# Ghostish/Open3DSOT

Measured on AMD Instinct MI355X. Metric: template/search pairs/sec (fwd+bwd), BAT KITTI-Car 512/1024 pts, higher is better.
Workload: dtype f32; 1 GPU; BAT_Car.yaml KITTI-Car, template 512 / search 1024 pts, batch 48 per GPU, fwd+bwd+Adam, fp32; global_batch=48, parallelism=dp1, fused_kernels=True, hip_graph=True, rccl_world_size=1

## Files before the change

### open3dsot_amd/csrc/compact.hip

```cpp
#include <cstdlib>
#include "o3d_common.hpp"

namespace {

__global__ __launch_bounds__(256) void compact_count_kernel(const int32_t* __restrict__ idx, long nslots, int ns,
                                                            int32_t* __restrict__ ball_cnt) {
    const long s = (long)blockIdx.x * 256 + threadIdx.x;
    const int lane = threadIdx.x & 63;
    const int v = s < nslots ? idx[s] : -1;
    const int base = lane & ~(ns - 1), k = lane - base;
    const int first = __shfl(v, base, 64);
    const unsigned long long m = __ballot(v != first);
    const unsigned long long seg = ns == 64 ? ~0ull : (((1ull << ns) - 1) << base);
    const unsigned long long other = m & seg;
    if (k == 0 && s < nslots) ball_cnt[s / ns] = other ? (63 - __clzll((long long)other)) - base + 1 : 1;
}

__global__ __launch_bounds__(1024) void compact_scan_kernel(const int32_t* __restrict__ ball_cnt, int n,
                                                            int col_base, int32_t* __restrict__ ball_off,
                                                            int32_t* __restrict__ meta) {
    __shared__ int sh[1024];
    const int per = (n + 1023) / 1024;
    const int i0 = threadIdx.x * per;
    int local = 0;
    for (int i = i0; i < i0 + per && i < n; ++i) local += ball_cnt[i];
    sh[threadIdx.x] = local;
    __syncthreads();
    for (int off = 1; off < 1024; off <<= 1) {
        const int v = (int)threadIdx.x >= off ? sh[threadIdx.x - off] : 0;
        __syncthreads();
        sh[threadIdx.x] += v;
        __syncthreads();
    }
    int run = col_base + sh[threadIdx.x] - local;
    for (int i = i0; i < i0 + per && i < n; ++i) {
        ball_off[i] = run;
        run += ball_cnt[i];
    }
    if (threadIdx.x == 1023) {
        const int tot = sh[1023];
        meta[0] = (tot + 255) & ~255;
        meta[1] = tot;
        meta[2] = n;
        meta[3] = 0;
    }
}

__global__ __launch_bounds__(256) void compact_fill_kernel(const int32_t* __restrict__ idx, long nslots, int ns,
                                                           int npoint, int ld, int col_base, int pt_base,
                                                           int ball_base, int dummy_ball,
                                                           const int32_t* __restrict__ ball_cnt,
                                                           const int32_t* __restrict__ ball_off,
                                                           const int32_t* __restrict__ meta,
                                                           int32_t* __restrict__ gp, int32_t* __restrict__ cball,
                                                           float* __restrict__ cw) {
    if (blockIdx.x == gridDim.x - 1) {
        const int q = meta[1] + threadIdx.x;
        if (q < meta[0]) { gp[col_base + q] = 0; cball[col_base + q] = dummy_ball; cw[col_base + q] = 0.f; }
        return;
    }
    const long s = (long)blockIdx.x * 256 + threadIdx.x;
    if (s >= nslots) return;
    const int ball = (int)(s / ns), k = (int)(s - (long)ball * ns);
    const int cnt = ball_cnt[ball];
    if (k >= cnt) return;
    const int q = ball_off[ball] + k;
    gp[q] = pt_base + (ball / npoint) * ld + idx[s];
    cball[q] = ball_base + ball;
    cw[q] = k == 0 ? (float)(1 + ns - cnt) : 1.f;
}

template <bool CENTERS, bool DIRECT = false>
__global__ __launch_bounds__(256) void expand_c_kernel(const float* __restrict__ Z, long ldz,
                                                       const int32_t* __restrict__ gp,
                                                       const int32_t* __restrict__ cball,
                                                       const float* __restrict__ cw,
                                                       const float* __restrict__ centers,
                                                       const float* __restrict__ W0, int ldw, int C0,
                                                       const int32_t* __restrict__ meta, long start1, long ldp,
                                                       float* __restrict__ Y0, float* __restrict__ part,
                                                       const float* __restrict__ stat_c) {
    const int q0 = blockIdx.x * 256;
    const int seg = (start1 > 0 && q0 >= start1) ? 1 : 0;
// ... 78 lines not shown
}

template <int POOL_CH>
__global__ __launch_bounds__(256) void pool_c_kernel(const float* __restrict__ Y, long ldp,
                                                     const float* __restrict__ scale,
                                                     const float* __restrict__ shift,
                                                     const int32_t* __restrict__ ball_off,
                                                     const int32_t* __restrict__ ball_cnt, int C, int seg1_ball,
                                                     int np0, int np1, int nballs, float* __restrict__ out,
                                                     int32_t* __restrict__ argq, float* __restrict__ yarg) {
    const int e = threadIdx.x & 7;
    int ball = blockIdx.x * 32 + (threadIdx.x >> 3);
    const bool live = ball < nballs;
    if (!live) ball = nballs - 1;
    const int q0 = ball_off[ball], q1 = q0 + ball_cnt[ball];
    const int c0 = blockIdx.y * POOL_CH;
    if (ball >= seg1_ball) { scale += C; shift += C; }
    constexpr int PU = 4;
    float v[POOL_CH][PU], sc[POOL_CH], sf[POOL_CH];
#pragma unroll
    for (int cc = 0; cc < POOL_CH; ++cc) {
        const int c = c0 + cc < C ? c0 + cc : C - 1;
        const float* y = Y + (long)c * ldp;
#pragma unroll
        for (int i = 0; i < PU; ++i) {
            const int q = q0 + e + 8 * i;
            v[cc][i] = y[q < q1 ? q : q1 - 1];
        }
        sc[cc] = scale[c];
        sf[cc] = shift[c];
    }
    float rbest[POOL_CH], ryb[POOL_CH];
    int rbq[POOL_CH];
#pragma unroll
    for (int cc = 0; cc < POOL_CH; ++cc) {
        float best = -INFINITY, yb = 0.f;
        int bq = 0x7fffffff;
#pragma unroll
        for (int i = 0; i < PU; ++i) {
            const int q = q0 + e + 8 * i;
            const float n = fmaf(v[cc][i], sc[cc], sf[cc]);
            if (q < q1 && n > best) { best = n; bq = q; yb = v[cc][i]; }
        }
        if (q1 - q0 > 8 * PU) {
            const float* y = Y + (long)(c0 + cc < C ? c0 + cc : C - 1) * ldp;
            for (int q = q0 + e + 8 * PU; q < q1; q += 8) {
                const float w = y[q], n = fmaf(w, sc[cc], sf[cc]);
                if (n > best) { best = n; bq = q; yb = w; }
            }
        }
        {
            const float ob = dpp_f<0xB1>(best), oy = dpp_f<0xB1>(yb);
            const int oq = dpp_i<0xB1>(bq);
            if (ob > best || (ob == best && oq < bq)) { best = ob; bq = oq; yb = oy; }
        }
        {
            const float ob = dpp_f<0x4E>(best), oy = dpp_f<0x4E>(yb);
            const int oq = dpp_i<0x4E>(bq);
            if (ob > best || (ob == best && oq < bq)) { best = ob; bq = oq; yb = oy; }
        }
        {
            const float ob = dpp_f<0x141>(best), oy = dpp_f<0x141>(yb);
            const int oq = dpp_i<0x141>(bq);
            if (ob > best || (ob == best && oq < bq)) { best = ob; bq = oq; yb = oy; }
        }
        rbest[cc] = best; ryb[cc] = yb; rbq[cc] = bq;
    }
    if (live && e == 0) {
#pragma unroll
        for (int cc = 0; cc < POOL_CH; ++cc) {
            const int c = c0 + cc;
            if (c < C) {
                const long o = pool_index(c, ball, C, seg1_ball, np0, np1);
                out[o] = fmaxf(rbest[cc], 0.f);
                if (argq) { argq[o] = rbq[cc]; yarg[o] = ryb[cc]; }
            }
        }
    }
}

constexpr int PT_CH = 32, PT_COLS = 128, PT_OVER = 32, PT_LD = PT_COLS + PT_OVER + 3;
constexpr int PT_RB = 32, PT_RLD = PT_CH + 1;

__device__ __forceinline__ void pool_t_item(const float* __restrict__ Y, long ldp,
                                            const float* __restrict__ scale, const float* __restrict__ shift,
                                            const int32_t* __restrict__ ball_off,
                                            const int32_t* __restrict__ ball_cnt,
                                            const int32_t* __restrict__ cball,
                                            const int32_t* __restrict__ meta, long start1, int C,
                                            int seg1_ball, int np0, int np1, int nballs,
                                            float* __restrict__ out, int32_t* __restrict__ argq,
                                            float* __restrict__ yarg, const long q0, const int c0, float* pt_tile) {
    int* pt_off = reinterpret_cast<int*>(pt_tile + PT_CH * PT_LD);
    int* pt_cnt = pt_off + PT_COLS;
    int* pt_ob = pt_cnt + PT_COLS;
    float* pt_res = reinterpret_cast<float*>(pt_ob + PT_COLS);
    const int seg = (start1 > 0 && q0 >= start1) ? 1 : 0;
    const long sbase = seg ? start1 : 0;
    if (q0 - sbase >= meta[4 * seg]) return;
    const long qend = sbase + meta[4 * seg + 1];
    if (q0 >= qend) return;
    int bfirst = cball[q0];
    if (ball_off[bfirst] < q0) ++bfirst;
    const long qlast = (q0 + PT_COLS < qend ? q0 + PT_COLS : qend) - 1;
    const int blast = cball[qlast];
    const int nb = blast - bfirst + 1;
    const int np = seg ? np1 : np0;
    const long segbase = seg ? (long)seg1_ball * C : 0;
    const int ball0 = seg ? seg1_ball : 0;
    constexpr int F4 = (PT_COLS + PT_OVER) / 4;
    constexpr int NLD = PT_CH * F4 / 256;
    static_assert(PT_CH * F4 % 256 == 0, "tile loads must divide evenly over the workgroup");
    {
        float4 v[NLD];
        int bo = 0, bc = 0;
        if ((int)threadIdx.x < nb) { bo = ball_off[bfirst + threadIdx.x]; bc = ball_cnt[bfirst + threadIdx.x]; }
#pragma unroll
        for (int u = 0; u < NLD; ++u) {
            const int i = threadIdx.x + 256 * u;
            const int r = i / F4, f = i - r * F4;
            long q = q0 + 4 * f;
            if (q + 4 > ldp) q = ldp - 4;
            v[u] = *reinterpret_cast<const float4*>(&Y[(long)(c0 + r) * ldp + q]);
        }
        __builtin_amdgcn_sched_barrier(0);
#pragma unroll
        for (int u = 0; u < NLD; ++u) {
            const int i = threadIdx.x + 256 * u;
            const int r = i / F4, f = i - r * F4;
            float* d = &pt_tile[r * PT_LD + 4 * f];
            d[0] = v[u].x; d[1] = v[u].y; d[2] = v[u].z; d[3] = v[u].w;
        }
        if ((int)threadIdx.x < PT_COLS) {
            const int local = bfirst + (int)threadIdx.x - ball0;
            const int b = local / np, j = local - b * np;
            pt_off[threadIdx.x] = bo;
            pt_cnt[threadIdx.x] = bc;
            pt_ob[threadIdx.x] = (int)(segbase + (long)b * C * np + j);
        }
    }
    const int lane = threadIdx.x & 63, wave = threadIdx.x >> 6;
    const int ch = lane & (PT_CH - 1), half = lane / PT_CH;
    constexpr int BPW = 64 / PT_CH;
    const float sc = scale[seg * C + c0 + ch], sf = shift[seg * C + c0 + ch];
    __syncthreads();
    const float* row = &pt_tile[ch * PT_LD];
    const int wj = threadIdx.x & 31, wc = threadIdx.x >> 5;
    for (int j0 = 0; j0 < nb; j0 += PT_RB) {
#pragma unroll 1
        for (int t = 0; t < PT_RB / 4; t += BPW) {
            const int jl = j0 + wave * (PT_RB / 4) + t + half;
            if (jl - half >= nb) break;
            const bool has = jl < nb;
            const int off = has ? pt_off[jl] : 0, cnt = has ? pt_cnt[jl] : 0;
            const int rel = (int)(off - q0);
            float best = -INFINITY, yb = 0.f;
            int bq = 0x7fffffff;
            for (int k = 0; k < cnt; k += 4) {
                const float w0 = row[rel + k], w1 = row[rel + k + 1], w2 = row[rel + k + 2], w3 = row[rel + k + 3];
                const float n0 = fmaf(w0, sc, sf), n1 = fmaf(w1, sc, sf), n2 = fmaf(w2, sc, sf), n3 = fmaf(w3, sc, sf);
                if (n0 > best) { best = n0; bq = off + k; yb = w0; }
                if (k + 1 < cnt && n1 > best) { best = n1; bq = off + k + 1; yb = w1; }
                if (k + 2 < cnt && n2 > best) { best = n2; bq = off + k + 2; yb = w2; }
                if (k + 3 < cnt && n3 > best) { best = n3; bq = off + k + 3; yb = w3; }
            }
            if (has) {
                float* r = &pt_res[(jl - j0) * PT_RLD + ch];
                r[0] = fmaxf(best, 0.f);
                r[PT_RB * PT_RLD] = __int_as_float(bq);
                r[2 * PT_RB * PT_RLD] = yb;
            }
        }
        __syncthreads();
        if (j0 + wj < nb) {
            const int ob = pt_ob[j0 + wj];
#pragma unroll
            for (int cc = wc; cc < PT_CH; cc += 8) {
                const long o = (long)ob + (long)(c0 + cc) * np;
                const float* r = &pt_res[wj * PT_RLD + cc];
                out[o] = r[0];
                if (argq) { argq[o] = __float_as_int(r[PT_RB * PT_RLD]); yarg[o] = r[2 * PT_RB * PT_RLD]; }
            }
        }
        __syncthreads();
    }
}

constexpr int PT_GRID = 4096;
__global__ __launch_bounds__(256) void pool_t_kernel(const float* __restrict__ Y, long ldp,
                                                     const float* __restrict__ scale, const float* __restrict__ shift,
                                                     const int32_t* __restrict__ ball_off,
                                                     const int32_t* __restrict__ ball_cnt,
                                                     const int32_t* __restrict__ cball,
                                                     const int32_t* __restrict__ meta, long start1, int C,
                                                     int seg1_ball, int np0, int np1, int nballs,
                                                     float* __restrict__ out, int32_t* __restrict__ argq,
                                                     float* __restrict__ yarg) {
    extern __shared__ float pt_tile[];
    const int ngrp = C / PT_CH;
    const int n0 = (meta[1] + PT_COLS - 1) / PT_COLS;
    const int n1 = start1 > 0 ? (meta[5] + PT_COLS - 1) / PT_COLS : 0;
    const long items = (long)(n0 + n1) * ngrp;
    for (long it = blockIdx.x; it < items; it += gridDim.x) {
        const int ch = (int)(it / ngrp), cg = (int)(it - (long)ch * ngrp);
        const long q0 = ch < n0 ? (long)ch * PT_COLS : start1 + (long)(ch - n0) * PT_COLS;
        pool_t_item(Y, ldp, scale, shift, ball_off, ball_cnt, cball, meta, start1, C, seg1_ball, np0, np1, nballs, out, argq, yarg, q0,
                    cg * PT_CH, pt_tile);
        __syncthreads();
    }
}

__global__ __launch_bounds__(256) void zero_cols_kernel(float* __restrict__ D, long ldp,
                                                        const int32_t* __restrict__ meta, long start1) {
    const long q = ((long)blockIdx.x * 256 + threadIdx.x) * 4;
    if (q >= ldp) return;
    const int seg = (start1 > 0 && q >= start1) ? 1 : 0;
    if (q - (seg ? start1 : 0) >= meta[4 * seg]) return;
    *reinterpret_cast<float4*>(&D[(long)blockIdx.y * ldp + q]) = make_float4(0.f, 0.f, 0.f, 0.f);
}

__global__ __launch_bounds__(256) void pool_bwd_partials_c_kernel(const float* __restrict__ dOut,
                                                                  const float* __restrict__ out,
                                                                  const float* __restrict__ yarg,
                                                                  const float* __restrict__ mean, int C,
                                                                  int nballs, int seg1_ball, int np0, int np1,
                                                                  float* __restrict__ part,
                                                                  const int32_t* __restrict__ argq,
                                                                  float* __restrict__ D, long ldp) {
    __shared__ float sh[2][4];
    const int c = blockIdx.x, seg = blockIdx.y, k = blockIdx.z;
    const int s0 = seg ? seg1_ball : 0, s1 = seg ? nballs : seg1_ball;
    const int share = (s1 - s0 + POOL_BWD_SPLIT - 1) / POOL_BWD_SPLIT;
    const int b0 = s0 + k * share, b1 = min(b0 + share, s1);
    const float mu = mean[seg * C + c];
    float s = 0.f, q = 0.f;
    for (int ball = b0 + threadIdx.x; ball < b1; ball += 256) {
        const long o = pool_index(c, ball, C, seg1_ball, np0, np1);
        const bool pos = out[o] > 0.f;
        const float g = pos ? dOut[o] : 0.f;
        if (D && pos) D[(long)c * ldp + argq[o]] = g;
        s += g;
        q += g * (yarg[o] - mu);
    }
#pragma unroll
    for (int m = 32; m >= 1; m >>= 1) { s += __shfl_xor(s, m, 64); q += __shfl_xor(q, m, 64); }
    if ((threadIdx.x & 63) == 0) { sh[0][threadIdx.x >> 6] = s; sh[1][threadIdx.x >> 6] = q; }
    __syncthreads();
    if (threadIdx.x == 0) {
        const long row = (long)seg * POOL_BWD_SPLIT + k;
        part[(row * 2 + 0) * C + c] = (sh[0][0] + sh[0][1]) + (sh[0][2] + sh[0][3]);
        part[(row * 2 + 1) * C + c] = (sh[1][0] + sh[1][1]) + (sh[1][2] + sh[1][3]);
    }
}

constexpr int PBD_COLS = 512, PBD_CH = 8, PBD_BALLS = 128, PBD_GRID = 4096;

struct PoolGrad { const float* p; long sb, sc; };

struct PoolBwdDense {
    PoolGrad g0, g1;
    const float* out; const int32_t* argq; const float* yarg; const float* mean; const int32_t* cball; const int32_t* ball_off;
    const int32_t* meta; long start1, ldp; int C, dummy_ball, seg1_ball, np0, np1;
    float* D; float* part;
};

__device__ __forceinline__ void pool_bwd_dense_item(const PoolBwdDense& a, const long q0, const int c0, float2 (&stg)[PBD_CH][PBD_BALLS],
                                                    int& sh_hi) {
    const PoolGrad g0 = a.g0, g1 = a.g1;
    const float* __restrict__ out = a.out; const int32_t* __restrict__ argq = a.argq; const float* __restrict__ yarg = a.yarg;
    const float* __restrict__ mean = a.mean; const int32_t* __restrict__ cball = a.cball;
    const int32_t* __restrict__ ball_off = a.ball_off; const int32_t* __restrict__ meta = a.meta;
    const long start1 = a.start1, ldp = a.ldp;
    const int C = a.C, dummy_ball = a.dummy_ball, seg1_ball = a.seg1_ball, np0 = a.np0, np1 = a.np1;
    float* __restrict__ D = a.D; float* __restrict__ part = a.part;
    const long chunk = q0 / PBD_COLS;
    const int seg = (start1 > 0 && q0 >= start1) ? 1 : 0;
    const long local0 = q0 - (seg ? start1 : 0);
    const int qi = threadIdx.x & 127, half = threadIdx.x >> 7;
    const long q = q0 + 4 * qi;
    const int live = meta[4 * seg];
    const int b_lo = cball[q0];
    const int4 cb = *reinterpret_cast<const int4*>(&cball[q]);
    if (threadIdx.x == 0) sh_hi = -1;
    if (local0 >= live) return;
    const int ncols = (int)min((long)PBD_COLS, live - local0);
    const bool mine = 4 * qi < ncols;
    __syncthreads();
    if (half == 0) {
        int hi = cb.x;
        hi = cb.y != dummy_ball ? cb.y : hi;
        hi = cb.z != dummy_ball ? cb.z : hi;
// ... 341 lines not shown
        if (T)
            for (int j = threadIdx.x; j < npoint; j += 256) {
                const int b0 = ball_off[bbase + j], b1 = b0 + ball_cnt[bbase + j];
                const int s0 = b0 > lo ? b0 : lo, s1 = b1 < hi ? b1 : hi;
                if (s0 >= s1) continue;
                float t[CS];
#pragma unroll
                for (int c = 0; c < CS; ++c) t[c] = 0.f;
                for (int q = s0; q < s1; ++q)
#pragma unroll
                    for (int c = 0; c < CS; ++c) t[c] += dy[c * CH + (q - lo)];
#pragma unroll
                for (int c = 0; c < CS; ++c) tacc[c * npoint + j] += t[c];
            }
    }
    __syncthreads();
    for (int i = threadIdx.x; i < CS * ld; i += 256) {
        const int c = i / ld, n = i - c * ld;
        if (c0 + c < C0) S[(long)(c0 + c) * lds_row + pbase + n] = sacc[i];
    }
    if (T)
        for (int i = threadIdx.x; i < CS * npoint; i += 256) {
            const int c = i / npoint, j = i - c * npoint;
            if (c0 + c < C0) T[(long)(c0 + c) * nballs + bbase + j] = tacc[i];
        }
}

__global__ __launch_bounds__(1024) void center_term_kernel(const float* __restrict__ T,
                                                           const float* __restrict__ centers, int nballs, int ldw,
                                                           float* __restrict__ dW, float* __restrict__ out = nullptr,
                                                           int ncols = 0) {
    __shared__ float red[16][3];
    const int c = blockIdx.x, tid = threadIdx.x;
    const float* t = T + (long)c * nballs;
    float s0 = 0.f, s1 = 0.f, s2 = 0.f;
    for (int ball = tid; ball < nballs; ball += 1024) {
        const float v = t[ball];
        s0 = fmaf(v, centers[3 * ball], s0);
        s1 = fmaf(v, centers[3 * ball + 1], s1);
        s2 = fmaf(v, centers[3 * ball + 2], s2);
    }
#pragma unroll
    for (int off = 32; off >= 1; off >>= 1) {
        s0 += __shfl_xor(s0, off, 64);
        s1 += __shfl_xor(s1, off, 64);
        s2 += __shfl_xor(s2, off, 64);
    }
    if ((tid & 63) == 0) { red[tid >> 6][0] = s0; red[tid >> 6][1] = s1; red[tid >> 6][2] = s2; }
    __syncthreads();
    if (tid < 3) {
        float a = 0.f;
#pragma unroll
        for (int w = 0; w < 16; ++w) a += red[w][tid];
        if (out) out[(long)c * ncols + tid] = dW[(long)c * ldw + tid] - a;
        else dW[(long)c * ldw + tid] -= a;
    }
    if (out)
        for (int k = 3 + tid; k < ncols; k += 1024) out[(long)c * ncols + k] = dW[(long)c * ldw + k];
}

struct PackSeg { const float* xyz; const float* feats; int N, ld; };

__global__ __launch_bounds__(256) void pack_points_kernel(PackSeg s0, PackSeg s1, int B, int nxyz, int C, float inv_radius,
                                                          long ldz, float* __restrict__ X0) {
    const long col = (long)blockIdx.x * 256 + threadIdx.x;
    if (col >= ldz) return;
    const int r = blockIdx.y;
    const long base1 = (long)B * s0.ld;
    const bool second = col >= base1;
    const PackSeg sg = second ? s1 : s0;
    const long local = second ? col - base1 : col;
    const int b = (int)(local / sg.ld), n = (int)(local - (long)b * sg.ld);
    float v = 0.f;
    if (n < sg.N) {
        if (r < nxyz) v = sg.xyz[((long)b * sg.N + n) * 3 + r] * inv_radius;
        else if (r < nxyz + C) v = sg.feats[((long)b * C + (r - nxyz)) * sg.N + n];
    }
    X0[(long)r * ldz + col] = v;
}

}

static bool pow2(int v) { return v > 0 && (v & (v - 1)) == 0; }
constexpr long O3D_MAX_BALLS = 1L << 20;

extern "C" int o3d_compact_build(const int32_t* idx, int B, int npoint, int ns, int ld, int col_base, int pt_base,
                                 int ball_base, int dummy_ball, int32_t* ball_cnt, int32_t* ball_off, int32_t* gp,
                                 int32_t* cball, float* cw, int32_t* meta, void* stream) {
    const long nballs = (long)B * npoint, nslots = nballs * ns;
    if (!idx || !ball_cnt || !ball_off || !gp || !cball || !cw || !meta || B <= 0 || npoint <= 0 || ns < 1 ||
        ns > 64 || !pow2(ns) || nballs > O3D_MAX_BALLS || nslots % 256 != 0 || ld <= 0 || col_base < 0 || col_base % 256 != 0)
        return O3D_EINVAL;
    hipStream_t s = o3d_stream(stream);
    const int blocks = (int)(nslots / 256);
    hipLaunchKernelGGL(compact_count_kernel, dim3(blocks), dim3(256), 0, s, idx, nslots, ns, ball_cnt);
    hipLaunchKernelGGL(compact_scan_kernel, dim3(1), dim3(1024), 0, s, ball_cnt, (int)nballs, col_base, ball_off, meta);
    hipLaunchKernelGGL(compact_fill_kernel, dim3(blocks + 1), dim3(256), 0, s, idx, nslots, ns, npoint, ld, col_base,
                       pt_base, ball_base, dummy_ball, ball_cnt, ball_off, meta, gp, cball, cw);
    return o3d_launch_status();
}

namespace {
template <int CPW>
__global__ __launch_bounds__(256) void dw0_xyz_kernel(const float* __restrict__ dN, const float* __restrict__ Y0, long ldp,
                                                      const float* __restrict__ A1, const float* __restrict__ A2,
                                                      const float* __restrict__ A3, const int32_t* __restrict__ gp,
                                                      const int32_t* __restrict__ cball, const float* __restrict__ cw,
                                                      const float* __restrict__ X, long ldz,
                                                      const float* __restrict__ centers,
                                                      const int32_t* __restrict__ meta, long start1, int C0,
                                                      float* __restrict__ part) {
    const long q0 = (long)blockIdx.x * 256;
    const int seg = (start1 > 0 && q0 >= start1) ? 1 : 0;
    float* prow = part + (long)blockIdx.x * C0 * 3;
    if (q0 - (seg ? start1 : 0) >= meta[4 * seg]) {
        for (int i = threadIdx.x; i < C0 * 3; i += 256) prow[i] = 0.f;
        return;
    }
    const int lane = threadIdx.x & 63, wave = threadIdx.x >> 6;
    const long q = q0 + 4 * lane;
    const int4 id = *reinterpret_cast<const int4*>(&gp[q]);
    const int4 bj = *reinterpret_cast<const int4*>(&cball[q]);
    const float4 w = *reinterpret_cast<const float4*>(&cw[q]);
    const int ids[4] = {id.x, id.y, id.z, id.w}, bb[4] = {bj.x, bj.y, bj.z, bj.w};
    const float wv[4] = {w.x, w.y, w.z, w.w};
    float rel[4][3];
#pragma unroll
    for (int t = 0; t < 4; ++t)
#pragma unroll
        for (int k = 0; k < 3; ++k)
            rel[t][k] = wv[t] != 0.f ? X[(long)k * ldz + ids[t]] - centers[(long)bb[t] * 3 + k] : 0.f;
    const float* a1 = A1 + seg * C0;
    const float* a2 = A2 + seg * C0;
    const float* a3 = A3 + seg * C0;
    for (int cbase = 0; cbase < C0; cbase += 4 * CPW) {
        float acc[CPW][3];
        float4 d[CPW], y[CPW];
#pragma unroll
        for (int i = 0; i < CPW; ++i) {
            const int c = cbase + wave + 4 * i;
            const int cc = c < C0 ? c : C0 - 1;
            d[i] = *reinterpret_cast<const float4*>(&dN[(long)cc * ldp + q]);
            y[i] = *reinterpret_cast<const float4*>(&Y0[(long)cc * ldp + q]);
        }
#pragma unroll
        for (int i = 0; i < CPW; ++i) {
            const int c = cbase + wave + 4 * i;
            const int cc = c < C0 ? c : C0 - 1;
            const float k1 = a1[cc], k2 = a2[cc], k3 = a3[cc];
            const float dv[4] = {d[i].x, d[i].y, d[i].z, d[i].w}, yv[4] = {y[i].x, y[i].y, y[i].z, y[i].w};
            float s0 = 0.f, s1 = 0.f, s2 = 0.f;
#pragma unroll
            for (int t = 0; t < 4; ++t) {
                const float dy = wv[t] != 0.f ? fmaf(k1, dv[t], wv[t] * fmaf(k2, yv[t], k3)) : 0.f;
                s0 = fmaf(dy, rel[t][0], s0); s1 = fmaf(dy, rel[t][1], s1); s2 = fmaf(dy, rel[t][2], s2);
            }
            acc[i][0] = s0; acc[i][1] = s1; acc[i][2] = s2;
        }
#pragma unroll
        for (int i = 0; i < CPW; ++i) {
            const int c = cbase + wave + 4 * i;
#pragma unroll
            for (int k = 0; k < 3; ++k) {
                const float t = wave_sum(acc[i][k]);
                if (lane == 0 && c < C0) prow[c * 3 + k] = t;
            }
// ... 92 lines not shown
        return;
    }
    const long s = (long)blk * 256 + threadIdx.x;
    if (s >= sg.nslots) return;
    const int ball = (int)(s / ns), k = (int)(s - (long)ball * ns);
    const int cnt = sg.ball_cnt[ball];
    if (k >= cnt) return;
    const int q = sg.ball_off[ball] + k;
    gp[q] = sg.pt_base + (ball / sg.npoint) * sg.ld + sg.idx[s];
    cball[q] = sg.ball_base + ball;
    cw[q] = k == 0 ? (float)(1 + ns - cnt) : 1.f;
}
}

extern "C" int o3d_compact_build2(const int32_t* idx0, int npoint0, int ld0, const int32_t* idx1, int npoint1, int ld1,
                                  int B, int ns, int col_base1, int pt_base1, int dummy_ball, int32_t* ball_cnt,
                                  int32_t* ball_off, int32_t* gp, int32_t* cball, float* cw, int32_t* meta, void* stream) {
    const long nb0 = (long)B * npoint0, nb1 = (long)B * npoint1;
    if (!idx0 || !idx1 || !ball_cnt || !ball_off || !gp || !cball || !cw || !meta || B <= 0 || npoint0 <= 0 ||
        npoint1 <= 0 || ns < 1 || ns > 64 || !pow2(ns) || nb0 > O3D_MAX_BALLS || nb1 > O3D_MAX_BALLS || (nb0 * ns) % 256 != 0 ||
        (nb1 * ns) % 256 != 0 || ld0 <= 0 || ld1 <= 0 || col_base1 < 0 || col_base1 % 256 != 0 || pt_base1 < 0)
        return O3D_EINVAL;
    CompactSeg s0 = {idx0, nb0 * ns, npoint0, ld0, 0, 0, 0, (int)nb0, ball_cnt, ball_off, meta};
    CompactSeg s1 = {idx1, nb1 * ns, npoint1, ld1, col_base1, pt_base1, (int)nb0, (int)nb1, ball_cnt + nb0, ball_off + nb0,
                     meta + 4};
    hipStream_t s = o3d_stream(stream);
    const int b0 = (int)(s0.nslots / 256), b1 = (int)(s1.nslots / 256);
    hipLaunchKernelGGL(compact_count2_kernel, dim3(b0 + b1), dim3(256), 0, s, s0, s1, ns, b0);
    hipLaunchKernelGGL(compact_scan2_kernel, dim3(2), dim3(1024), 0, s, s0, s1);
    hipLaunchKernelGGL(compact_fill2_kernel, dim3(b0 + b1 + 2), dim3(256), 0, s, s0, s1, ns, b0, dummy_ball, gp, cball, cw);
    return o3d_launch_status();
}

extern "C" int o3d_group_expand_c(const float* Z, long ldz, const int32_t* gp, const int32_t* cball,
                                  const float* cw, const float* centers, const float* W0, int ldw, int C0,
                                  const int32_t* meta, long start1, long ldp, float* Y0, float* part,
                                  const float* stat_c, void* stream) {
    if (!Z || !gp || !cball || !cw || !meta || !Y0 || C0 <= 0 || ldp <= 0 || ldp % 256 != 0 || start1 < 0 ||
        start1 % 256 != 0 || (centers && (!W0 || ldw < 3)))
        return O3D_EINVAL;
    const int ysplit = C0 >= 128 ? 4 : C0 >= 64 ? 2 : 1;
    if (centers)
        hipLaunchKernelGGL(expand_c_kernel<true>, dim3((unsigned)(ldp / 256), ysplit), dim3(256), 0, o3d_stream(stream), Z,
                           ldz, gp, cball, cw, centers, W0, ldw, C0, meta, start1, ldp, Y0, part, stat_c);
    else
        hipLaunchKernelGGL(expand_c_kernel<false>, dim3((unsigned)(ldp / 256), ysplit), dim3(256), 0, o3d_stream(stream), Z,
                           ldz, gp, cball, cw, centers, W0, ldw, C0, meta, start1, ldp, Y0, part, stat_c);
    return o3d_launch_status();
}

extern "C" int o3d_group_expand_c3(const float* X3, long ldz, const int32_t* gp, const int32_t* cball, const float* cw,
                                   const float* centers, const float* W0, int ldw, int C0, const int32_t* meta,
                                   long start1, long ldp, float* Y0, float* part, const float* stat_c, void* stream) {
    if (!X3 || !gp || !cball || !cw || !centers || !W0 || ldw < 3 || !meta || !Y0 || C0 <= 0 || ldp <= 0 ||
        ldp % 256 != 0 || start1 < 0 || start1 % 256 != 0)
        return O3D_EINVAL;
    const int ysplit = C0 >= 128 ? 4 : C0 >= 64 ? 2 : 1;
    hipLaunchKernelGGL((expand_c_kernel<true, true>), dim3((unsigned)(ldp / 256), ysplit), dim3(256), 0, o3d_stream(stream),
                       X3, ldz, gp, cball, cw, centers, W0, ldw, C0, meta, start1, ldp, Y0, part, stat_c);
    return o3d_launch_status();
}

extern "C" int o3d_pool_fwd_c(const float* Y, long ldp, const float* scale, const float* shift,
                              const int32_t* ball_off, const int32_t* ball_cnt, int B, int C, int npoint0,
                              int npoint1, float* out, int32_t* argq, float* yarg, void* stream) {
    if (!Y || !scale || !shift || !ball_off || !ball_cnt || !out || B <= 0 || C <= 0 || npoint0 <= 0 || npoint1 < 0 ||
        (argq && !yarg))
        return O3D_EINVAL;
    const int seg1_ball = B * npoint0, nballs = B * (npoint0 + npoint1);
    constexpr int POOL_CH = 8;
    hipLaunchKernelGGL(pool_c_kernel<8>, dim3(o3d_cdiv(nballs, 32), o3d_cdiv(C, POOL_CH)), dim3(256), 0,
                       o3d_stream(stream), Y, ldp, scale, shift, ball_off, ball_cnt, C, seg1_ball, npoint0,
                       npoint1 > 0 ? npoint1 : npoint0, nballs, out, argq, yarg);
    return o3d_launch_status();
}

extern "C" int o3d_pool_fwd_ct(const float* Y, long ldp, const float* scale, const float* shift, const int32_t* ball_off,
                               const int32_t* ball_cnt, const int32_t* cball, const int32_t* meta, long start1, int B, int C,
                               int npoint0, int npoint1, int nsample, float* out, int32_t* argq, float* yarg, void* stream) {
    if (!Y || !scale || !shift || !ball_off || !ball_cnt || !cball || !meta || !out || B <= 0 || C <= 0 || C % PT_CH != 0 ||
        npoint0 <= 0 || npoint1 < 0 || nsample < 1 || nsample > PT_OVER || (argq && !yarg) || ldp < PT_COLS + PT_OVER ||
        ldp % PT_COLS != 0 || start1 < 0 || start1 % PT_COLS != 0)
        return O3D_EINVAL;
    const int seg1_ball = B * npoint0, nballs = B * (npoint0 + npoint1);
    const size_t lds = sizeof(float) * (PT_CH * PT_LD + 3 * PT_RB * PT_RLD) + sizeof(int) * 3 * PT_COLS;
    static const bool attr_ok = hipFuncSetAttribute(reinterpret_cast<const void*>(pool_t_kernel),
                                                    hipFuncAttributeMaxDynamicSharedMemorySize, (int)lds) == hipSuccess;
    if (!attr_ok) return O3D_ELAUNCH;
    const long worst = (ldp / PT_COLS) * (C / PT_CH);
    hipLaunchKernelGGL(pool_t_kernel, dim3((unsigned)(worst < PT_GRID ? worst : PT_GRID)), dim3(256), lds, o3d_stream(stream), Y, ldp,
                       scale, shift, ball_off, ball_cnt, cball, meta, start1, C, seg1_ball, npoint0,
                       npoint1 > 0 ? npoint1 : npoint0, nballs, out, argq, yarg);
    return o3d_launch_status();
}

extern "C" int o3d_pool_bwd_c(const float* dOut, const float* out, const int32_t* argq, const float* yarg,
                              const float* mean, int B, int C, int npoint0, int npoint1, const int32_t* meta,
                              long start1, long ldp, float* D, float* part, void* stream) {
    if (!dOut || !out || !argq || !yarg || !mean || !meta || !D || !part || B <= 0 || C <= 0 || npoint0 <= 0 ||
        npoint1 < 0 || ldp <= 0 || ldp % 4 != 0)
        return O3D_EINVAL;
    hipStream_t s = o3d_stream(stream);
    const int nseg = npoint1 > 0 ? 2 : 1;
    const int seg1_ball = B * npoint0, nballs = B * (npoint0 + npoint1), np1 = npoint1 > 0 ? npoint1 : npoint0;
    hipLaunchKernelGGL(zero_cols_kernel, dim3((unsigned)o3d_cdiv(ldp, 1024), C), dim3(256), 0, s, D, ldp, meta, start1);
    hipLaunchKernelGGL(pool_bwd_partials_c_kernel, dim3(C, nseg, POOL_BWD_SPLIT), dim3(256), 0, s, dOut, out, yarg, mean, C,
                       nballs, seg1_ball, npoint0, np1, part, argq, D, ldp);
    return o3d_launch_status();
}

extern "C" int o3d_pool_bwd_dense(const float* dOut0, long sb0, long sc0, const float* dOut1, long sb1, long sc1,
                                  const float* out, const int32_t* argq, const float* yarg,
                                  const float* mean, const int32_t* cball, const int32_t* ball_off, const int32_t* meta,
                                  long start1, long ldp, int B, int C, int npoint0, int npoint1, float* D, float* part,
                                  void* stream) {
    if (!out || !argq || !yarg || !mean || !cball || !ball_off || !meta || !D || !part || B <= 0 || C <= 0 ||
        C % PBD_CH != 0 || npoint0 <= 0 || npoint1 < 0 || ldp <= 0 || ldp % PBD_COLS != 0 || start1 < 0 ||
        start1 % PBD_COLS != 0 || ldp > 0x7fffffffL)
        return O3D_EINVAL;
    const int seg1_ball = B * npoint0, np1 = npoint1 > 0 ? npoint1 : npoint0;
    const PoolGrad g0 = {dOut0, sb0, sc0}, g1 = {dOut1, sb1, sc1};
    PoolBwdDense a = {g0, g1, out, argq, yarg, mean, cball, ball_off, meta, npoint1 > 0 ? start1 : 0, ldp, C,
                      B * (npoint0 + npoint1), seg1_ball, npoint0, np1, D, part};
    const long worst = (ldp / PBD_COLS) * (C / PBD_CH);
    const unsigned grid = (unsigned)(worst < PBD_GRID ? worst : PBD_GRID);
    hipLaunchKernelGGL(pool_bwd_dense_kernel, dim3(grid), dim3(256), 0, o3d_stream(stream), a);
    return o3d_launch_status();
}

template <int CS, int BT = 256>
static int launch_reduce_c(const float* dN, const float* Y0, long ldp, const float* A1, const float* A2,
                           const float* A3, const int32_t* gp, const int32_t* cball, const float* cw,
                           const int32_t* ball_off, const int32_t* ball_cnt, int B, int nseg, SegParams sp0,
                           SegParams sp1, int C0,
                           long lds_row, int nballs, float* S, float* T, hipStream_t s) {
    const int span = (sp0.ld + sp0.npoint) > (sp1.ld + sp1.npoint) ? (sp0.ld + sp0.npoint) : (sp1.ld + sp1.npoint);
    const size_t lds = sizeof(float) * CS * (size_t)span;
    if (lds > 64 * 1024) return O3D_EINVAL;
    if (lds > 48 * 1024 &&
        hipFuncSetAttribute(reinterpret_cast<const void*>(reduce_c_kernel<CS, BT>),
                            hipFuncAttributeMaxDynamicSharedMemorySize, (int)lds) != hipSuccess)
        return O3D_ELAUNCH;
    const int slabs = (C0 + CS - 1) / CS;
    hipLaunchKernelGGL((reduce_c_kernel<CS, BT>), dim3(B * nseg * slabs), dim3(BT), lds, s, dN, Y0, ldp, A1, A2, A3, gp, cball,
                       cw, ball_off, ball_cnt, B, sp0, sp1, C0, lds_row, S, T, nballs);
    return o3d_launch_status();
}

extern "C" int o3d_group_reduce_c(const float* dN, const float* Y0, long ldp, const float* A1, const float* A2,
                                  const float* A3, const int32_t* gp, const int32_t* cball, const float* cw,
                                  const int32_t* ball_off, const int32_t* ball_cnt, int B, int nseg, int npoint0,
                                  int ld0, int npoint1, int ld1, int C0, float* S, float* T, void* stream) {
    if (!dN || !Y0 || !A1 || !A2 || !A3 || !gp || !cball || !cw || !ball_off || !ball_cnt || !S || B <= 0 || npoint0 <= 0 ||
        ld0 <= 0 || C0 <= 0 || (nseg != 1 && nseg != 2) || (nseg == 2 && (npoint1 <= 0 || ld1 <= 0)))
        return O3D_EINVAL;
    hipStream_t s = o3d_stream(stream);
    const SegParams sp0 = {npoint0, ld0, 0, 0};
    const SegParams sp1 = nseg == 2 ? SegParams{npoint1, ld1, B * ld0, B * npoint0} : sp0;
    const long lds_row = (long)B * ld0 + (nseg == 2 ? (long)B * ld1 : 0);
    const int nballs = B * npoint0 + (nseg == 2 ? B * npoint1 : 0);
    return launch_reduce_c<1>(dN, Y0, ldp, A1, A2, A3, gp, cball, cw, ball_off, ball_cnt, B, nseg, sp0, sp1, C0,
                              lds_row, nballs, S, T, s);
}

extern "C" int o3d_center_term(const float* T, const float* centers, int C0, int nballs, int ldw, float* dW,
                               void* stream) {
    if (!T || !centers || !dW || C0 <= 0 || nballs <= 0 || ldw < 3) return O3D_EINVAL;
    hipLaunchKernelGGL(center_term_kernel, dim3(C0), dim3(1024), 0, o3d_stream(stream), T, centers, nballs, ldw, dW,
                       static_cast<float*>(nullptr), 0);
    return o3d_launch_status();
}

extern "C" int o3d_center_term_out(const float* T, const float* centers, int C0, int nballs, int ldw, const float* dW,
                                   int ncols, float* out, void* stream) {
    if (!T || !centers || !dW || !out || C0 <= 0 || nballs <= 0 || ncols < 3 || ldw < ncols) return O3D_EINVAL;
// ... 93 lines not shown
```

Before: 9119 pairs/s.

## Software-pipeline pool_t tile loads across persistent items with occupancy-sized grid

Restructures the transposed pooling kernel into a persistent loop that prefetches the next work item's tile, scale/shift and ball metadata into registers while the current item is reduced from LDS. It also remaps block indices so neighbouring items are spread across XCDs, and sizes the grid to the number of resident workgroups from an occupancy query instead of a fixed cap. The aim is to hide global load latency and cut tail imbalance, at the cost of more register pressure from the held prefetch.

Measured after the change: 9129 pairs/s (median of 4 runs). About the same (+0.1%).

```diff
diff --git a/open3dsot_amd/csrc/compact.hip b/open3dsot_amd/csrc/compact.hip
--- a/open3dsot_amd/csrc/compact.hip
+++ b/open3dsot_amd/csrc/compact.hip
@@ -1,4 +1,5 @@
 #include <cstdlib>
+#include <mutex>
 #include "o3d_common.hpp"
 
 namespace {
@@ -243,131 +244,146 @@
 constexpr int PT_CH = 32, PT_COLS = 128, PT_OVER = 32, PT_LD = PT_COLS + PT_OVER + 3;
 constexpr int PT_RB = 32, PT_RLD = PT_CH + 1;
 
-__device__ __forceinline__ void pool_t_item(const float* __restrict__ Y, long ldp,
-                                            const float* __restrict__ scale, const float* __restrict__ shift,
-                                            const int32_t* __restrict__ ball_off,
-                                            const int32_t* __restrict__ ball_cnt,
-                                            const int32_t* __restrict__ cball,
-                                            const int32_t* __restrict__ meta, long start1, int C,
-                                            int seg1_ball, int np0, int np1, int nballs,
-                                            float* __restrict__ out, int32_t* __restrict__ argq,
-                                            float* __restrict__ yarg, const long q0, const int c0, float* pt_tile) {
-    int* pt_off = reinterpret_cast<int*>(pt_tile + PT_CH * PT_LD);
-    int* pt_cnt = pt_off + PT_COLS;
-    int* pt_ob = pt_cnt + PT_COLS;
-    float* pt_res = reinterpret_cast<float*>(pt_ob + PT_COLS);
-    const int seg = (start1 > 0 && q0 >= start1) ? 1 : 0;
-    const long sbase = seg ? start1 : 0;
-    if (q0 - sbase >= meta[4 * seg]) return;
-    const long qend = sbase + meta[4 * seg + 1];
-    if (q0 >= qend) return;
-    int bfirst = cball[q0];
-    if (ball_off[bfirst] < q0) ++bfirst;
+__device__ __forceinline__ int xcd_order(int x, int G) { return G % 8 == 0 ? (x % 8) * (G / 8) + x / 8 : x; }
+
+constexpr int PT_F4 = (PT_COLS + PT_OVER) / 4;
+constexpr int PT_NLD = PT_CH * PT_F4 / 256;
+static_assert(PT_CH * PT_F4 % 256 == 0, "tile loads must divide evenly over the workgroup");
+
+struct PtItem {
+    float4 v[PT_NLD];
+    int bo, bc;
+    int bfirst, nb;
+    float sc, sf;
+};
+
+__device__ __forceinline__ void pt_coords(long it, int ngrp, int n0, long start1, long& q0, int& c0, int& seg) {
+    const int ch = (int)(it / ngrp), cg = (int)(it - (long)ch * ngrp);
+    seg = ch < n0 ? 0 : 1;
+    q0 = seg ? start1 + (long)(ch - n0) * PT_COLS : (long)ch * PT_COLS;
+    c0 = cg * PT_CH;
+}
+
+__device__ __forceinline__ void pt_fetch(PtItem& p, long it, int ngrp, int n0, long start1, const int live[2],
+                                         const float* __restrict__ Y, long ldp, const float* __restrict__ scale,
+                                         const float* __restrict__ shift, const int32_t* __restrict__ ball_off,
+                                         const int32_t* __restrict__ ball_cnt, const int32_t* __restrict__ cball, int C) {
+    long q0;
+    int c0, seg;
+    pt_coords(it, ngrp, n0, start1, q0, c0, seg);
+    const long sbase = seg ? start1 : 0, qend = sbase + live[seg];
     const long qlast = (q0 + PT_COLS < qend ? q0 + PT_COLS : qend) - 1;
+    const bool at_start = q0 == sbase;
+    const int cprev = cball[at_start ? q0 : q0 - 1];
     const int blast = cball[qlast];
-    const int nb = blast - bfirst + 1;
-    const int np = seg ? np1 : np0;
-    const long segbase = seg ? (long)seg1_ball * C : 0;
-    const int ball0 = seg ? seg1_ball : 0;
-    constexpr int F4 = (PT_COLS + PT_OVER) / 4;
-    constexpr int NLD = PT_CH * F4 / 256;
-    static_assert(PT_CH * F4 % 256 == 0, "tile loads must divide evenly over the workgroup");
-    {
-        float4 v[NLD];
-        int bo = 0, bc = 0;
-        if ((int)threadIdx.x < nb) { bo = ball_off[bfirst + threadIdx.x]; bc = ball_cnt[bfirst + threadIdx.x]; }
-#pragma unroll
-        for (int u = 0; u < NLD; ++u) {
-            const int i = threadIdx.x + 256 * u;
-            const int r = i / F4, f = i - r * F4;
-            long q = q0 + 4 * f;
-            if (q + 4 > ldp) q = ldp - 4;
-            v[u] = *reinterpret_cast<const float4*>(&Y[(long)(c0 + r) * ldp + q]);
-        }
-        __builtin_amdgcn_sched_barrier(0);
-#pragma unroll
-        for (int u = 0; u < NLD; ++u) {
-            const int i = threadIdx.x + 256 * u;
-            const int r = i / F4, f = i - r * F4;
-            float* d = &pt_tile[r * PT_LD + 4 * f];
-            d[0] = v[u].x; d[1] = v[u].y; d[2] = v[u].z; d[3] = v[u].w;
-        }
-        if ((int)threadIdx.x < PT_COLS) {
-            const int local = bfirst + (int)threadIdx.x - ball0;
-            const int b = local / np, j = local - b * np;
-            pt_off[threadIdx.x] = bo;
-            pt_cnt[threadIdx.x] = bc;
-            pt_ob[threadIdx.x] = (int)(segbase + (long)b * C * np + j);
-        }
-    }
-    const int lane = threadIdx.x & 63, wave = threadIdx.x >> 6;
-    const int ch = lane & (PT_CH - 1), half = lane / PT_CH;
-    constexpr int BPW = 64 / PT_CH;
-    const float sc = scale[seg * C + c0 + ch], sf = shift[seg * C + c0 + ch];
-    __syncthreads();
-    const float* row = &pt_tile[ch * PT_LD];
-    const int wj = threadIdx.x & 31, wc = threadIdx.x >> 5;
-    for (int j0 = 0; j0 < nb; j0 += PT_RB) {
-#pragma unroll 1
-        for (int t = 0; t < PT_RB / 4; t += BPW) {
-            const int jl = j0 + wave * (PT_RB / 4) + t + half;
-            if (jl - half >= nb) break;
-            const bool has = jl < nb;
-            const int off = has ? pt_off[jl] : 0, cnt = has ? pt_cnt[jl] : 0;
-            const int rel = (int)(off - q0);
-            float best = -INFINITY, yb = 0.f;
-            int bq = 0x7fffffff;
-            for (int k = 0; k < cnt; k += 4) {
-                const float w0 = row[rel + k], w1 = row[rel + k + 1], w2 = row[rel + k + 2], w3 = row[rel + k + 3];
-                const float n0 = fmaf(w0, sc, sf), n1 = fmaf(w1, sc, sf), n2 = fmaf(w2, sc, sf), n3 = fmaf(w3, sc, sf);
-                if (n0 > best) { best = n0; bq = off + k; yb = w0; }
-                if (k + 1 < cnt && n1 > best) { best = n1; bq = off + k + 1; yb = w1; }
-                if (k + 2 < cnt && n2 > best) { best = n2; bq = off + k + 2; yb = w2; }
-                if (k + 3 < cnt && n3 > best) { best = n3; bq = off + k + 3; yb = w3; }
-            }
-            if (has) {
-                float* r = &pt_res[(jl - j0) * PT_RLD + ch];
-                r[0] = fmaxf(best, 0.f);
-                r[PT_RB * PT_RLD] = __int_as_float(bq);
-                r[2 * PT_RB * PT_RLD] = yb;
-            }
-        }
-        __syncthreads();
-        if (j0 + wj < nb) {
-            const int ob = pt_ob[j0 + wj];
-#pragma unroll
-            for (int cc = wc; cc < PT_CH; cc += 8) {
-                const long o = (long)ob + (long)(c0 + cc) * np;
-                const float* r = &pt_res[wj * PT_RLD + cc];
-                out[o] = r[0];
-                if (argq) { argq[o] = __float_as_int(r[PT_RB * PT_RLD]); yarg[o] = r[2 * PT_RB * PT_RLD]; }
-            }
-        }
-        __syncthreads();
-    }
-}
-
-constexpr int PT_GRID = 4096;
+    __builtin_amdgcn_sched_barrier(0);
+    const int ch = threadIdx.x & (PT_CH - 1);
+    p.sc = scale[seg * C + c0 + ch];
+    p.sf = shift[seg * C + c0 + ch];
+#pragma unroll
+    for (int u = 0; u < PT_NLD; ++u) {
+        const int i = threadIdx.x + 256 * u;
+        const int r = i / PT_F4, f = i - r * PT_F4;
+        long q = q0 + 4 * f;
+        if (q + 4 > ldp) q = ldp - 4;
+        p.v[u] = *reinterpret_cast<const float4*>(&Y[(long)(c0 + r) * ldp + q]);
+    }
+    __builtin_amdgcn_sched_barrier(0);
+    p.bfirst = at_start ? cprev : cprev + 1;
+    p.nb = blast - p.bfirst + 1;
+    p.bo = 0; p.bc = 0;
+    if ((int)threadIdx.x < p.nb) { p.bo = ball_off[p.bfirst + threadIdx.x]; p.bc = ball_cnt[p.bfirst + threadIdx.x]; }
+}
+
 __global__ __launch_bounds__(256) void pool_t_kernel(const float* __restrict__ Y, long ldp,
                                                      const float* __restrict__ scale, const float* __restrict__ shift,
                                                      const int32_t* __restrict__ ball_off,
                                                      const int32_t* __restrict__ ball_cnt,
                                                      const int32_t* __restrict__ cball,
                                                      const int32_t* __restrict__ meta, long start1, int C,
-                                                     int seg1_ball, int np0, int np1, int nballs,
+                                                     int seg1_ball, int np0, int np1,
                                                      float* __restrict__ out, int32_t* __restrict__ argq,
                                                      float* __restrict__ yarg) {
     extern __shared__ float pt_tile[];
+    int* pt_off = reinterpret_cast<int*>(pt_tile + PT_CH * PT_LD);
+    int* pt_cnt = pt_off + PT_COLS;
+    int* pt_ob = pt_cnt + PT_COLS;
+    float* pt_res = reinterpret_cast<float*>(pt_ob + PT_COLS);
     const int ngrp = C / PT_CH;
-    const int n0 = (meta[1] + PT_COLS - 1) / PT_COLS;
-    const int n1 = start1 > 0 ? (meta[5] + PT_COLS - 1) / PT_COLS : 0;
+    const int live[2] = {meta[1], start1 > 0 ? meta[5] : 0};
+    const int n0 = (live[0] + PT_COLS - 1) / PT_COLS, n1 = (live[1] + PT_COLS - 1) / PT_COLS;
     const long items = (long)(n0 + n1) * ngrp;
-    for (long it = blockIdx.x; it < items; it += gridDim.x) {
-        const int ch = (int)(it / ngrp), cg = (int)(it - (long)ch * ngrp);
-        const long q0 = ch < n0 ? (long)ch * PT_COLS : start1 + (long)(ch - n0) * PT_COLS;
-        pool_t_item(Y, ldp, scale, shift, ball_off, ball_cnt, cball, meta, start1, C, seg1_ball, np0, np1, nballs, out, argq, yarg, q0,
-                    cg * PT_CH, pt_tile);
+    long it = xcd_order(blockIdx.x, gridDim.x);
+    if (it >= items) return;
+    PtItem p;
+    pt_fetch(p, it, ngrp, n0, start1, live, Y, ldp, scale, shift, ball_off, ball_cnt, cball, C);
+    const int lane = threadIdx.x & 63, wave = threadIdx.x >> 6;
+    const int ch = lane & (PT_CH - 1), half = lane / PT_CH;
+    constexpr int BPW = 64 / PT_CH;
+    const float* row = &pt_tile[ch * PT_LD];
+    const int wj = threadIdx.x & 31, wc = threadIdx.x >> 5;
+    for (; it < items; it += gridDim.x) {
+        long q0;
+        int c0, seg;
+        pt_coords(it, ngrp, n0, start1, q0, c0, seg);
+        const int nb = p.nb;
+        const float sc = p.sc, sf = p.sf;
+        const int np = seg ? np1 : np0;
+#pragma unroll
+        for (int u = 0; u < PT_NLD; ++u) {
+            const int i = threadIdx.x + 256 * u;
+            const int r = i / PT_F4, f = i - r * PT_F4;
+            float* d = &pt_tile[r * PT_LD + 4 * f];
+            d[0] = p.v[u].x; d[1] = p.v[u].y; d[2] = p.v[u].z; d[3] = p.v[u].w;
+        }
+        if ((int)threadIdx.x < PT_COLS) {
+            const int local = p.bfirst + (int)threadIdx.x - (seg ? seg1_ball : 0);
+            const int b = local / np, j = local - b * np;
+            pt_off[threadIdx.x] = p.bo;
+            pt_cnt[threadIdx.x] = p.bc;
+            pt_ob[threadIdx.x] = (int)((seg ? (long)seg1_ball * C : 0) + (long)b * C * np + j);
+        }
+        if (it + gridDim.x < items)
+            pt_fetch(p, it + gridDim.x, ngrp, n0, start1, live, Y, ldp, scale, shift, ball_off, ball_cnt, cball, C);
         __syncthreads();
+        for (int j0 = 0; j0 < nb; j0 += PT_RB) {
+#pragma unroll 1
+            for (int t = 0; t < PT_RB / 4; t += BPW) {
+                const int jl = j0 + wave * (PT_RB / 4) + t + half;
+                if (jl - half >= nb) break;
+                const bool has = jl < nb;
+                const int off = has ? pt_off[jl] : 0, cnt = has ? pt_cnt[jl] : 0;
+                const int rel = (int)(off - q0);
+                float best = -INFINITY, yb = 0.f;
+                int bq = 0x7fffffff;
+                for (int k = 0; k < cnt; k += 4) {
+                    const float w0 = row[rel + k], w1 = row[rel + k + 1], w2 = row[rel + k + 2], w3 = row[rel + k + 3];
+                    const float m0 = fmaf(w0, sc, sf), m1 = fmaf(w1, sc, sf), m2 = fmaf(w2, sc, sf), m3 = fmaf(w3, sc, sf);
+                    if (m0 > best) { best = m0; bq = off + k; yb = w0; }
+                    if (k + 1 < cnt && m1 > best) { best = m1; bq = off + k + 1; yb = w1; }
+                    if (k + 2 < cnt && m2 > best) { best = m2; bq = off + k + 2; yb = w2; }
+                    if (k + 3 < cnt && m3 > best) { best = m3; bq = off + k + 3; yb = w3; }
+                }
+                if (has) {
+                    float* r = &pt_res[(jl - j0) * PT_RLD + ch];
+                    r[0] = fmaxf(best, 0.f);
+                    r[PT_RB * PT_RLD] = __int_as_float(bq);
+                    r[2 * PT_RB * PT_RLD] = yb;
+                }
+            }
+            __syncthreads();
+            if (j0 + wj < nb) {
+                const int ob = pt_ob[j0 + wj];
+#pragma unroll
+                for (int cc = wc; cc < PT_CH; cc += 8) {
+                    const long o = (long)ob + (long)(c0 + cc) * np;
+                    const float* r = &pt_res[wj * PT_RLD + cc];
+                    out[o] = r[0];
+                    if (argq) { argq[o] = __float_as_int(r[PT_RB * PT_RLD]); yarg[o] = r[2 * PT_RB * PT_RLD]; }
+                }
+            }
+            __syncthreads();
+        }
     }
 }
 
@@ -875,6 +891,24 @@
 }
 
 static bool pow2(int v) { return v > 0 && (v & (v - 1)) == 0; }
+
+static long resident_wgs(const void* fn, size_t lds) {
+    struct Entry { int dev; const void* fn; size_t lds; long n; };
+    static Entry cache[32];
+    static int used = 0;
+    static std::mutex mu;
+    int dev = 0;
+    if (hipGetDevice(&dev) != hipSuccess) dev = 0;
+    std::lock_guard<std::mutex> lock(mu);
+    for (int i = 0; i < used; ++i)
+        if (cache[i].dev == dev && cache[i].fn == fn && cache[i].lds == lds) return cache[i].n;
+    int cus = 0, per_cu = 0;
+    if (hipDeviceGetAttribute(&cus, hipDeviceAttributeMultiprocessorCount, dev) != hipSuccess || cus <= 0) cus = 256;
+    if (hipOccupancyMaxActiveBlocksPerMultiprocessor(&per_cu, fn, 256, lds) != hipSuccess || per_cu <= 0) per_cu = 1;
+    const long n = (long)cus * per_cu;
+    if (used < 32) cache[used++] = {dev, fn, lds, n};
+    return n;
+}
 constexpr long O3D_MAX_BALLS = 1L << 20;
 
 extern "C" int o3d_compact_build(const int32_t* idx, int B, int npoint, int ns, int ld, int col_base, int pt_base,
@@ -1133,15 +1167,16 @@
         npoint0 <= 0 || npoint1 < 0 || nsample < 1 || nsample > PT_OVER || (argq && !yarg) || ldp < PT_COLS + PT_OVER ||
         ldp % PT_COLS != 0 || start1 < 0 || start1 % PT_COLS != 0)
         return O3D_EINVAL;
-    const int seg1_ball = B * npoint0, nballs = B * (npoint0 + npoint1);
+    const int seg1_ball = B * npoint0;
     const size_t lds = sizeof(float) * (PT_CH * PT_LD + 3 * PT_RB * PT_RLD) + sizeof(int) * 3 * PT_COLS;
     static const bool attr_ok = hipFuncSetAttribute(reinterpret_cast<const void*>(pool_t_kernel),
                                                     hipFuncAttributeMaxDynamicSharedMemorySize, (int)lds) == hipSuccess;
     if (!attr_ok) return O3D_ELAUNCH;
     const long worst = (ldp / PT_COLS) * (C / PT_CH);
-    hipLaunchKernelGGL(pool_t_kernel, dim3((unsigned)(worst < PT_GRID ? worst : PT_GRID)), dim3(256), lds, o3d_stream(stream), Y, ldp,
+    const long grid = resident_wgs(reinterpret_cast<const void*>(pool_t_kernel), lds);
+    hipLaunchKernelGGL(pool_t_kernel, dim3((unsigned)(worst < grid ? worst : grid)), dim3(256), lds, o3d_stream(stream), Y, ldp,
                        scale, shift, ball_off, ball_cnt, cball, meta, start1, C, seg1_ball, npoint0,
-                       npoint1 > 0 ? npoint1 : npoint0, nballs, out, argq, yarg);
+                       npoint1 > 0 ? npoint1 : npoint0, out, argq, yarg);
     return o3d_launch_status();
 }
 
```
